# caizexin/GenVC

Measured on AMD Instinct MI355X. Metric: utterances/s (streaming, 1 s chunks; with RTF and first-chunk latency), higher is better.
Workload: dtype f32; 1 GPU; GenVC_small streaming, 1 s chunks, top_k=1, batch 1 per GPU (BASELINE configs[1]); parallelism=replicas x1, utterances sharded by rank, all_gather of token ids

## Files before the change

genvc_amd/csrc/attn64.h:

```cpp
#pragma once
#include "gemm.h"

namespace gvc {

typedef float hb_f32x4 __attribute__((ext_vector_type(4)));

template <bool MASK, int NW = 4>
__global__ __launch_bounds__(NW * 64) void k_attn64_mfma(const float* qb, const float* kb, const float* vb, long long ld, long long bs, int Tq,
                                                     int Tk, float* out, int out_rows, int E, float scale, int out_fm16, const int32_t* fmask) {
    __shared__ float sm[NW][16], sl[NW][16];
    __shared__ __attribute__((aligned(16))) float so[NW][16][68];
    const int tid = threadIdx.x, lane = tid & 63, wave = tid >> 6, r = lane & 15, g = lane >> 4;
    const int q0 = blockIdx.x * 16, h = blockIdx.y, b = blockIdx.z;
    const float* base = qb + (size_t)b * bs + h * 64;
    const float* kbase = kb + (size_t)b * bs + h * 64;
    const float* vbase = vb + (size_t)b * bs + h * 64;
    const int T = Tk;
    const int qi = min(q0 + r, Tq - 1);
    float4 qf[4];
#pragma unroll
    for (int s = 0; s < 4; ++s) {
        qf[s] = *reinterpret_cast<const float4*>(base + (size_t)qi * ld + 16 * s + 4 * g);
        qf[s].x *= scale; qf[s].y *= scale; qf[s].z *= scale; qf[s].w *= scale;
    }
// ... 58 lines not shown
        *reinterpret_cast<float4*>(&so[wave][r][16 * g + 4 * i]) = make_float4(o[0][i], o[1][i], o[2][i], o[3][i]);
    __syncthreads();
    const int qr = tid >> 4, dc = (tid & 15) * 4;
    if (tid < 256 && q0 + qr < Tq) {
        float M = sm[0][qr];
#pragma unroll
        for (int w = 1; w < NW; ++w) M = fmaxf(M, sm[w][qr]);
        float L = 0.f;
        float4 acc = make_float4(0.f, 0.f, 0.f, 0.f);
#pragma unroll
        for (int w = 0; w < NW; ++w) {
            const float f = sm[w][qr] == -INFINITY ? 0.f : expf(sm[w][qr] - M);
            L += sl[w][qr] * f;
            const float4 ov = *reinterpret_cast<const float4*>(&so[w][qr][dc]);
            acc.x += ov.x * f; acc.y += ov.y * f; acc.z += ov.z * f; acc.w += ov.w * f;
        }
        const float inv = 1.0f / L;
        acc.x *= inv; acc.y *= inv; acc.z *= inv; acc.w *= inv;
        if (out_fm16) *reinterpret_cast<float4*>(out + fm16_index(b * out_rows + q0 + qr, h * 64 + dc, E)) = acc;
        else *reinterpret_cast<float4*>(out + ((size_t)b * out_rows + q0 + qr) * E + h * 64 + dc) = acc;
    }
}

}
```

genvc_amd/csrc/gemm.h:

```cpp
#pragma once
#include "common.h"

namespace gvc {

__host__ __device__ __forceinline__ size_t fm16_index(int m, int k, int K) {
    return ((size_t)(m >> 4) * (K >> 4) + (k >> 4)) * 256 + (size_t)((((m & 15) + 16 * ((k & 15) >> 2)) << 2) + (k & 3));
}

enum GemmAct { ACT_NONE = 0, ACT_GELU_NEW = 1, ACT_RELU = 2, ACT_GELU_ERF = 3 };
enum GemmAAct { AACT_NONE = 0, AACT_LRELU = 1 };

struct GemmEpi {
    const float* bias;
    long long bias_batch_stride;
    int act;
    const float* resid;
    int ldr;
    long long resid_batch_stride;
    long long resid_batch_stride2;
    int resid_fm16;
    int geglu;
    const float* resid2;
    float out_scale;
    int c_fm16;
// ... 188 lines not shown
    *reinterpret_cast<float4*>(G.C + (size_t)m * G.ldc + n) = v;
}

typedef float f32x16 __attribute__((ext_vector_type(16)));

__global__ __launch_bounds__(256) void k_gemm_f32(const GemmArgs G);
__global__ void k_splitk_epilogue(const GemmArgs G);

int launch_gemm_skinny(GemmArgs G, int SK, long long work_cap, hipStream_t s);
int launch_ln_sum_rows(const float* x_in, float* x_out, float* a, const float* part, int SK, const float* bias, int rows, int d,
                       const float* ln_w, const float* ln_b, int a_fm16, hipStream_t s);
struct LnFuse {
    const float* x_in; float* x_out;
    const float* part; int SK; const float* pbias;
    const float* ln_w; const float* ln_b;
    int rows;
};
int launch_gemm_skinny_ln(GemmArgs G, const LnFuse& P, hipStream_t s);
int launch_gemm_strip(GemmArgs G, int sk_max, long long work_cap, int raw_partials, int* sk_used, hipStream_t s);
void gemm_init_attributes();
__global__ void k_to_fm16(const float* src, float* dst, int N, int K);
__global__ void k_to_fm16_bf16(const float* src, unsigned short* dst, int N, int K);

int launch_gemm_cap(GemmArgs G, int batch, long long work_cap, hipStream_t s);

}
```

genvc_amd/csrc/gemm.hip:

```cpp
#include "gemm.h"
#include "gemm_b16.h"
#include <algorithm>

namespace gvc {

constexpr int BM = 64, BN = 64, BK = 32, LDL = 36;

__global__ __launch_bounds__(256) void k_gemm_f32(const GemmArgs G) {
    __shared__ __attribute__((aligned(16))) float As[2][BM * LDL];
    __shared__ __attribute__((aligned(16))) float Bs[2][BN * LDL];
    const int tid = threadIdx.x, lane = tid & 63, wave = tid >> 6;
    const int wm = wave >> 1, wn = wave & 1;
    const int batch = blockIdx.z / G.SK, sk = blockIdx.z - batch * G.SK;
    const int m0 = blockIdx.y * BM, n0 = blockIdx.x * BN;
    const int ntile_all = (G.K + BK - 1) / BK;
    const int tps = (ntile_all + G.SK - 1) / G.SK;
    const int kbeg = sk * tps * BK;
    const int kend = min(G.K, kbeg + tps * BK);
    const int nt = kend > kbeg ? (kend - kbeg + BK - 1) / BK : 0;
    const float* Ab = G.A + gemm_boff(G, batch, G.a_batch_stride, G.a_batch_stride2);
    const float* Wb = G.Wt + gemm_binner(G, batch) * G.w_batch_stride;

    float4 ra[2], rb[2];
    auto load_tile = [&](int kt) {
// ... 64 lines not shown
                G.work[(((size_t)batch * G.SK + sk) * G.M + m) * G.N + n] = acc[r];
            else
                gemm_store(G, batch, m, n, acc[r]);
        }
    }
}

__global__ void k_splitk_epilogue(const GemmArgs G) {
    const int batch = blockIdx.z;
    const size_t mn = (size_t)G.M * G.N;
    for (size_t i = (size_t)blockIdx.x * blockDim.x + threadIdx.x; i < mn; i += (size_t)gridDim.x * blockDim.x) {
        const float* w = G.work + (size_t)batch * G.SK * mn + i;
        float pv[16];
#pragma unroll
        for (int s = 0; s < 16; ++s) pv[s] = w[(size_t)min(s, G.SK - 1) * mn];
        float v = 0.f;
#pragma unroll
        for (int s = 0; s < 16; ++s)
            if (s < G.SK) v += pv[s];
        gemm_store(G, batch, (int)(i / G.N), (int)(i % G.N), v);
    }
}

int launch_gemm_cap(GemmArgs G, int batch, long long work_cap, hipStream_t s) {
    GVC_REQUIRE(G.K % 4 == 0 && G.lda % 4 == 0 && G.ldw % 4 == 0 && G.conv_cin % 4 == 0 && G.conv_tap_stride % 4 == 0,
                GVC_ERR_ARG, "gemm: K/lda/ldw/conv strides must be multiples of 4 (K=%d lda=%d ldw=%d)", G.K, G.lda, G.ldw);
    const int tm = cdiv(G.M, BM), tn = cdiv(G.N, BN);
    const long long tiles = (long long)tm * tn * batch;
    int SK = 1;
    constexpr int sk_tiles = 128, sk_target = 192;
    if (tiles < sk_tiles && G.work) {
        SK = (int)((sk_target + tiles - 1) / tiles);
        const int max_by_k = G.K / (4 * BK) > 0 ? G.K / (4 * BK) : 1;
        if (SK > max_by_k) SK = max_by_k;
        if (SK > 16) SK = 16;
        while (SK > 1 && (long long)batch * SK * G.M * G.N > work_cap) --SK;
    } else if (tiles < 2 * sk_tiles && G.K >= 64 * BK && G.work) {
        SK = (int)((4 * sk_tiles + tiles - 1) / tiles);
        if (SK > G.K / (16 * BK)) SK = G.K / (16 * BK);
        while (SK > 1 && (long long)batch * SK * G.M * G.N > work_cap) --SK;
    }
    G.SK = SK;
    dim3 grid(tn, tm, batch * SK);
    hipLaunchKernelGGL(k_gemm_f32, grid, dim3(256), 0, s, G);
    GVC_LAUNCH_CHECK();
    if (SK > 1) {
        const long long mn = (long long)G.M * G.N;
        int gx = (int)((mn + 255) / 256);
        if (gx > 2048) gx = 2048;
        hipLaunchKernelGGL(k_splitk_epilogue, dim3(gx, 1, batch), dim3(256), 0, s, G);
        GVC_LAUNCH_CHECK();
    }
    return GVC_OK;
}

typedef float f32x4 __attribute__((ext_vector_type(4)));

template <int WB> struct WRaw { typedef float4 T; };
template <> struct WRaw<1> { typedef uint2 T; };
__device__ __forceinline__ float4 w_f4(const float4& r) { return r; }
__device__ __forceinline__ float4 w_f4(const uint2& u) {
    return make_float4(__uint_as_float(u.x << 16), __uint_as_float(u.x & 0xffff0000u), __uint_as_float(u.y << 16),
                       __uint_as_float(u.y & 0xffff0000u));
}

template <int MT, int NW, int WB = 0, int NC = 0>
__global__ __launch_bounds__(NW * 64) void k_gemm_skinny(const GemmArgs G) {
    extern __shared__ __attribute__((aligned(16))) float red_raw[];
    float (*red)[MT][256] = reinterpret_cast<float (*)[MT][256]>(red_raw);
// ... 775 lines not shown
```

genvc_amd/csrc/hubert.hip:

```cpp
#include <map>
#include <string>
#include <vector>

#include "conv_lds.h"
#include "attn64.h"
#include <algorithm>

namespace gvc {

constexpr int kC0Chunk = 32;

static __global__ void k_hb_repack_conv(const float* w, float* out, int Co, int Ci, int k) {
    const size_t n = (size_t)Co * Ci * k;
    for (size_t i = (size_t)blockIdx.x * blockDim.x + threadIdx.x; i < n; i += (size_t)gridDim.x * blockDim.x) {
        const int j = (int)(i % k);
        const int ci = (int)((i / k) % Ci);
        const int co = (int)(i / ((size_t)k * Ci));
        out[((size_t)co * k + j) * Ci + ci] = w[i];
    }
}

static __global__ __launch_bounds__(256) void k_hb_conv0(const float* wav, const float* w, float* y, float* part, int T,
                                                        int T0, int C, int k, int stride) {
    extern __shared__ float xs[];
    const int b = blockIdx.z, chunk = blockIdx.x, tid = threadIdx.x;
    const int t0 = chunk * kC0Chunk;
    const int nt = min(kC0Chunk, T0 - t0);
    const int nx = (nt - 1) * stride + k;
    const float* src = wav + (size_t)b * T + (size_t)t0 * stride;
    for (int i = tid; i < nx; i += 256) xs[i] = src[i];
    __syncthreads();
    for (int c = blockIdx.y * 256 + tid; c < min(C, (int)(blockIdx.y + 1) * 256); c += 256) {
        float wr[16];
// ... 39 lines not shown
    const double mean = s / T0;
    double var = ss / T0 - mean * mean;
    if (var < 0.0) var = 0.0;
    stats[((size_t)b * C + c) * 2] = (float)mean;
    stats[((size_t)b * C + c) * 2 + 1] = (float)(1.0 / sqrt(var + 1e-5));
}

static __global__ void k_hb_gn_gelu(float* y, const float* stats, const float* gamma, const float* beta, int T0, int C) {
    const int b = blockIdx.y;
    const size_t n4 = (size_t)T0 * C / 4;
    float* yb = y + (size_t)b * T0 * C;
    for (size_t i = (size_t)blockIdx.x * blockDim.x + threadIdx.x; i < n4; i += (size_t)gridDim.x * blockDim.x) {
        const int c = (int)((i * 4) % C);
        float4 v = *reinterpret_cast<float4*>(yb + i * 4);
        const float* st = stats + ((size_t)b * C + c) * 2;
        v.x = gelu_erf((v.x - st[0]) * st[1] * gamma[c] + beta[c]);
        v.y = gelu_erf((v.y - st[2]) * st[3] * gamma[c + 1] + beta[c + 1]);
        v.z = gelu_erf((v.z - st[4]) * st[5] * gamma[c + 2] + beta[c + 2]);
        v.w = gelu_erf((v.w - st[6]) * st[7] * gamma[c + 3] + beta[c + 3]);
        *reinterpret_cast<float4*>(yb + i * 4) = v;
    }
}

static __global__ __launch_bounds__(256) void k_hb_ln_rows(const float* src, long long src_bs, float* dst, long long dst_bs,
                                                          int rpb, int d, const float* w, const float* b,
                                                          const float* part = nullptr, int SK = 0, const float* pbias = nullptr,
                                                          int rows = 0, float* dst_fm16 = nullptr) {
    __shared__ float red[4];
    const int row = blockIdx.x, tid = threadIdx.x;
    const int bi = row / rpb, ri = row - bi * rpb;
    const float* xr = src + bi * src_bs + (size_t)ri * d;
    float* orow = dst + bi * dst_bs + (size_t)ri * d;
    float4 v[4];
    float s = 0.f;
#pragma unroll
    for (int i = 0; i < 4; ++i) {
        const int k = (i * 256 + tid) * 4;
        v[i] = k < d ? *reinterpret_cast<const float4*>(xr + k) : make_float4(0.f, 0.f, 0.f, 0.f);
        if (part && k < d) {
            const float4 b4 = *reinterpret_cast<const float4*>(pbias + k);
            float4 p4[8];
#pragma unroll
            for (int sidx = 0; sidx < 8; ++sidx)
                p4[sidx] = *reinterpret_cast<const float4*>(part + ((size_t)min(sidx, SK - 1) * rows + row) * d + k);
            v[i].x += b4.x; v[i].y += b4.y; v[i].z += b4.z; v[i].w += b4.w;
#pragma unroll
            for (int sidx = 0; sidx < 8; ++sidx)
                if (sidx < SK) { v[i].x += p4[sidx].x; v[i].y += p4[sidx].y; v[i].z += p4[sidx].z; v[i].w += p4[sidx].w; }
        }
        s += (v[i].x + v[i].y) + (v[i].z + v[i].w);
    }
    const float inv_d = 1.0f / (float)d;
    const float mean = block4_sum(s, red) * inv_d;
    float q = 0.f;
#pragma unroll
    for (int i = 0; i < 4; ++i) {
        const int k = (i * 256 + tid) * 4;
        if (k < d) {
            const float a0 = v[i].x - mean, a1 = v[i].y - mean, a2 = v[i].z - mean, a3 = v[i].w - mean;
            q += (a0 * a0 + a1 * a1) + (a2 * a2 + a3 * a3);
        }
    }
    const float rstd = 1.0f / sqrtf(block4_sum(q, red) * inv_d + 1e-5f);
#pragma unroll
    for (int i = 0; i < 4; ++i) {
        const int k = (i * 256 + tid) * 4;
        if (k < d) {
            const float4 gw = *reinterpret_cast<const float4*>(w + k);
            const float4 gb = *reinterpret_cast<const float4*>(b + k);
            float4 o;
// ... 7 lines not shown

static __global__ void k_hb_zero_pad(float* buf, int C, int T, int front, int back, const int32_t* fmask) {
    const int b = blockIdx.y;
    float* base = buf + (size_t)b * (front + T + back) * C;
    const size_t nf = (size_t)front * C, nb = (size_t)back * C;
    for (size_t i = (size_t)blockIdx.x * blockDim.x + threadIdx.x; i < nf + nb; i += (size_t)gridDim.x * blockDim.x) {
        if (i < nf) base[i] = 0.f;
        else base[(size_t)(front + T) * C + (i - nf)] = 0.f;
    }
    for (int t = blockIdx.x; t < T; t += gridDim.x) {
        if (!fmask[b * T + t]) continue;
        for (int i = threadIdx.x; i < C; i += blockDim.x) base[(size_t)(front + t) * C + i] = 0.f;
    }
}

static __global__ __launch_bounds__(64) void k_hb_frame_mask(const float* wav, int32_t* fmask, int T, int F) {
    const int f = blockIdx.x, b = blockIdx.y, lane = threadIdx.x;
    const int chunk = T / F;
    const float* p = wav + (size_t)b * T + (size_t)f * chunk;
    int nz = 0;
    for (int i = lane; i < chunk; i += 64) nz |= (p[i] != 0.f);
    nz = __any(nz);
    if (lane == 0) fmask[b * F + f] = nz ? 0 : 1;
}

}

using namespace gvc;

struct HbLin { float* w = nullptr; float* b = nullptr; int N = 0, K = 0; float* wf = nullptr;  };
struct HbLn { float* w = nullptr; float* b = nullptr; };
struct HbLayer { HbLin qkv, out, fc1, fc2; HbLn ln1, ln2; };

struct gvc_hubert {
    gvc_hubert_dims dm;
    int cg = 0, pad_front = 0, pad_back = 0;
    float* conv0_w = nullptr;
    HbLn gn;
    std::vector<float*> conv_w;
    std::vector<float*> conv_wp;
    int conv_lds = 1;
    int conv_lds_rows = 256;
    HbLn feat_ln, enc_ln;
    HbLin proj, pos, fin;
    std::vector<HbLayer> layers;
    std::map<std::string, int> bound;
    int n_expected = 0;
    float *act[2] = {nullptr, nullptr};
    float *part = nullptr, *stats = nullptr;
    int32_t* fmask = nullptr;
    float *xp = nullptr, *x = nullptr, *qkv = nullptr, *att = nullptr, *hbuf = nullptr, *tmp = nullptr, *work = nullptr;
    long long work_cap = 0;
    int max_frames = 0, max_t0 = 0;
    std::map<long long, hipGraphExec_t> graphs;
    hipStream_t cap_stream = nullptr;
    int use_graph = 1;
    int skinny = 1;
    int strip = 1;
    bool fm_ready = false;
    float *xf = nullptr, *af = nullptr, *hf = nullptr;
    std::vector<void*> allocs;
};

static int hb_alloc(gvc_hubert* c, float** p, size_t n) {
    GVC_CHECK_HIP(hipMalloc((void**)p, n * sizeof(float)));
    c->allocs.push_back(*p);
    return GVC_OK;
}
static int hb_alloc_lin(gvc_hubert* c, HbLin& L, int N, int K) {
    L.N = N; L.K = K;
    int rc = hb_alloc(c, &L.w, (size_t)N * K);
    return rc ? rc : hb_alloc(c, &L.b, N);
}
static int hb_alloc_ln(gvc_hubert* c, HbLn& L, int d) {
    int rc = hb_alloc(c, &L.w, d);
    return rc ? rc : hb_alloc(c, &L.b, d);
}

static int hb_frames(const gvc_hubert_dims& D, int n, int upto) {
    for (int i = 0; i < upto; ++i) {
        if (n < D.conv_kernel[i]) return 0;
// ... 42 lines not shown
                conv_lds_bytes(D.conv_dim[i - 1], D.conv_kernel[i], 1, false, D.conv_stride[i]) <= kConvLdsMax)
                rc = hb_alloc(c, &wp, (size_t)D.conv_dim[i] * D.conv_kernel[i] * D.conv_dim[i - 1]);
            c->conv_wp.push_back(wp);
        }
    }
    const int Cl = D.conv_dim[D.n_conv - 1];
    if (!rc) rc = hb_alloc_ln(c, c->feat_ln, Cl);
    if (!rc) rc = hb_alloc_lin(c, c->proj, E, Cl);
    if (!rc) rc = hb_alloc_lin(c, c->pos, E, kp * c->cg);
    if (!rc) rc = hb_alloc_ln(c, c->enc_ln, E);
    c->layers.resize(D.n_layers);
    for (int l = 0; l < D.n_layers && !rc; ++l) {
        HbLayer& L = c->layers[l];
        if ((rc = hb_alloc_lin(c, L.qkv, 3 * E, E))) break;
        if ((rc = hb_alloc_lin(c, L.out, E, E))) break;
        if ((rc = hb_alloc_lin(c, L.fc1, D.ffn_dim, E))) break;
        if ((rc = hb_alloc_lin(c, L.fc2, E, D.ffn_dim))) break;
        if ((rc = hb_alloc_ln(c, L.ln1, E))) break;
        if ((rc = hb_alloc_ln(c, L.ln2, E))) break;
        for (HbLin* q : {&L.qkv, &L.out, &L.fc1, &L.fc2})
            if ((rc = hb_alloc(c, &q->wf, (size_t)q->N * q->K))) break;
    }
    if (!rc) rc = hb_alloc_lin(c, c->fin, D.final_dim, E);
    c->n_expected = 3 + (D.n_conv - 1) + 2 + 2 + 2 + 2 + 16 * D.n_layers + 2;
    const size_t B = D.max_batch, F = c->max_frames;
    for (int i = 0; i < 2 && !rc; ++i) rc = hb_alloc(c, &c->act[i], B * maxact);
    if (!rc) rc = hb_alloc(c, &c->part, B * (size_t)cdiv(c->max_t0, kC0Chunk) * D.conv_dim[0] * 2);
    if (!rc) rc = hb_alloc(c, &c->stats, B * D.conv_dim[0] * 2);
    if (!rc) rc = hb_alloc(c, reinterpret_cast<float**>(&c->fmask), B * F);
    if (!rc) rc = hb_alloc(c, &c->xp, B * (F + kp) * E);
    if (!rc) rc = hb_alloc(c, &c->x, B * F * E);
    if (!rc) rc = hb_alloc(c, &c->tmp, B * F * E);
    if (!rc) rc = hb_alloc(c, &c->att, B * F * E);
    if (!rc) rc = hb_alloc(c, &c->qkv, B * F * 3 * E);
    if (!rc) rc = hb_alloc(c, &c->hbuf, B * F * D.ffn_dim);
    const size_t fm_rows = std::max<size_t>(128, (B * F + 15) & ~(size_t)15);
    if (!rc) rc = hb_alloc(c, &c->xf, fm_rows * E);
    if (!rc) rc = hb_alloc(c, &c->af, fm_rows * E);
    if (!rc) rc = hb_alloc(c, &c->hf, fm_rows * D.ffn_dim);
    c->work_cap = 16ll << 20;
    if (!rc) rc = hb_alloc(c, &c->work, (size_t)c->work_cap);
    if (!rc && hipStreamCreateWithFlags(&c->cap_stream, hipStreamNonBlocking) != hipSuccess) rc = GVC_ERR_HIP;
    if (getenv("GVC_GRAPHS")) c->use_graph = atoi(getenv("GVC_GRAPHS"));
    conv_lds_init_attributes();
    if (E % 128 != 0 || D.ffn_dim % 128 != 0) c->skinny = 0;
    if (rc) { gvc_hubert_destroy(c); return rc; }
    *out = c;
    return GVC_OK;
}

extern "C" int gvc_hubert_destroy(gvc_hubert* c) {
    if (!c) return GVC_OK;
    for (auto& kv : c->graphs) hipGraphExecDestroy(kv.second);
    if (c->cap_stream) hipStreamDestroy(c->cap_stream);
    for (void* p : c->allocs) hipFree(p);
    delete c;
    return GVC_OK;
}

static int hb_copy(float* dst, const float* src, int64_t numel, int64_t expect, const char* name, hipStream_t s) {
    GVC_REQUIRE(numel == expect, GVC_ERR_ARG, "%s: expected %lld elements, got %lld", name, (long long)expect, (long long)numel);
    GVC_CHECK_HIP(hipMemcpyAsync(dst, src, numel * sizeof(float), hipMemcpyDeviceToDevice, s));
    return GVC_OK;
}

static bool ends_with(const std::string& n, const char* suf) {
// ... 42 lines not shown
        HbLayer& L = c->layers[l];
        const size_t dot = n.find('.', 15);
        const std::string sub = n.substr(dot + 1);
        int which = -1;
        if (sub.rfind("self_attn.q_proj.", 0) == 0) which = 0;
        else if (sub.rfind("self_attn.k_proj.", 0) == 0) which = 1;
        else if (sub.rfind("self_attn.v_proj.", 0) == 0) which = 2;
        if (which >= 0) {
            if (is_b) rc = hb_copy(L.qkv.b + (size_t)which * E, src, numel, E, name, s);
            else rc = hb_copy(L.qkv.w + (size_t)which * E * E, src, numel, (int64_t)E * E, name, s);
        } else if (sub.rfind("self_attn.out_proj.", 0) == 0) rc = lin(L.out);
        else if (sub.rfind("self_attn_layer_norm.", 0) == 0) rc = ln(L.ln1, E);
        else if (sub.rfind("fc1.", 0) == 0) rc = lin(L.fc1);
        else if (sub.rfind("fc2.", 0) == 0) rc = lin(L.fc2);
        else if (sub.rfind("final_layer_norm.", 0) == 0) rc = ln(L.ln2, E);
        else known = false;
    } else known = false;
    if (rc == GVC_OK && known) { c->bound[n] = 1; c->fm_ready = false; }
    return rc;
}

extern "C" int gvc_hubert_missing_weights(gvc_hubert* c) { return c ? c->n_expected - (int)c->bound.size() : -1; }

static int hb_linear(gvc_hubert* c, const HbLin& L, const float* A, float* C, int M, int act, const float* resid, hipStream_t s) {
    GemmArgs G;
    memset(&G, 0, sizeof(G));
    G.A = A; G.lda = L.K; G.Wt = L.w; G.ldw = L.K; G.C = C; G.ldc = L.N;
    G.M = M; G.N = L.N; G.K = L.K; G.work = c->work;
    G.e.bias = L.b; G.e.act = act;
    if (resid) { G.e.resid = resid; G.e.ldr = L.N; }
    return launch_gemm_cap(G, 1, c->work_cap, s);
}

static int hb_body(gvc_hubert* c, int B, int T, hipStream_t s) {
    const gvc_hubert_dims& D = c->dm;
    const int E = D.embed_dim;
    int rc;
    int Tin = hb_frames(D, T, 1);
    const int C0 = D.conv_dim[0];
    const int nchunk = cdiv(Tin, kC0Chunk);
    hipLaunchKernelGGL(k_hb_gn_stats, dim3(cdiv(C0, 8), B), dim3(256), 0, s, c->part, c->stats, nchunk, Tin, C0);
    GVC_LAUNCH_CHECK();
    {
        const size_t n4 = (size_t)Tin * C0 / 4;
        const int gx = (int)std::min<size_t>((n4 + 255) / 256, 4096);
        hipLaunchKernelGGL(k_hb_gn_gelu, dim3(gx, B), dim3(256), 0, s, c->act[0], c->stats, c->gn.w, c->gn.b, Tin, C0);
        GVC_LAUNCH_CHECK();
    }
    int cur = 0;
    for (int i = 1; i < D.n_conv; ++i) {
        const int Ci = D.conv_dim[i - 1], Co = D.conv_dim[i], k = D.conv_kernel[i], st = D.conv_stride[i];
        const int Tout = (Tin - k) / st + 1;
        if (c->conv_lds && c->conv_wp[i - 1] && Tout <= c->conv_lds_rows) {
            ConvLdsArgs A;
            memset(&A, 0, sizeof(A));
            A.x = c->act[cur]; A.x_bs = (long long)Tin * Ci; A.ldx = Ci; A.x_scale = 1.f; A.slope = 1.f;
            A.x_rows = Tin; A.stride = st;
            A.y = c->act[cur ^ 1]; A.y_bs = (long long)Tout * Co; A.ldy = Co;
            A.T = Tout; A.ntiles = Co / 16; A.act = ACT_GELU_ERF;
            A.job[0].wp = reinterpret_cast<const float4*>(c->conv_wp[i - 1]); A.job[0].k = k; A.job[0].dil = 1;
            if ((rc = launch_conv_lds(Ci, 1, A, 1, B, conv_lds_bytes(Ci, k, 1, false, st), s))) return rc;
            cur ^= 1;
            Tin = Tout;
            continue;
        }
        GemmArgs G;
        memset(&G, 0, sizeof(G));
        G.A = c->act[cur]; G.lda = st * Ci; G.a_batch_stride = (long long)Tin * Ci;
        G.Wt = c->conv_w[i - 1]; G.ldw = k * Ci;
        G.C = c->act[cur ^ 1]; G.ldc = Co; G.c_batch_stride = (long long)Tout * Co;
        G.M = Tout; G.N = Co; G.K = k * Ci; G.work = c->work;
        G.e.act = ACT_GELU_ERF;
        if ((rc = launch_gemm_cap(G, B, c->work_cap, s))) return rc;
        cur ^= 1;
        Tin = Tout;
    }
    const int F = Tin, Cl = D.conv_dim[D.n_conv - 1], rows = B * F;
    const int kp = D.pos_conv_kernel;
    const long long xp_bs = (long long)(F + kp - 1) * E;
    hipLaunchKernelGGL(k_hb_ln_rows, dim3(rows), dim3(256), 0, s, c->act[cur], (long long)F * Cl, c->act[cur ^ 1],
                       (long long)F * Cl, F, Cl, c->feat_ln.w, c->feat_ln.b);
    GVC_LAUNCH_CHECK();
    {
        GemmArgs G;
        memset(&G, 0, sizeof(G));
        G.A = c->act[cur ^ 1]; G.lda = Cl; G.a_batch_stride = (long long)F * Cl;
        G.Wt = c->proj.w; G.ldw = Cl;
        G.C = c->xp + (size_t)c->pad_front * E; G.ldc = E; G.c_batch_stride = xp_bs;
        G.M = F; G.N = E; G.K = Cl; G.work = c->work;
        G.e.bias = c->proj.b;
        if ((rc = launch_gemm_cap(G, B, c->work_cap, s))) return rc;
    }
    hipLaunchKernelGGL(k_hb_zero_pad, dim3(64, B), dim3(256), 0, s, c->xp, E, F, c->pad_front, c->pad_back, c->fmask);
    GVC_LAUNCH_CHECK();
    {
        GemmArgs G;
        memset(&G, 0, sizeof(G));
        const int cg = c->cg;
        G.batch_inner = D.pos_conv_groups;
        G.A = c->xp; G.lda = E; G.a_batch_stride = cg; G.a_batch_stride2 = xp_bs;
        G.conv_cin = cg; G.conv_tap_stride = E;
        G.Wt = c->pos.w; G.ldw = kp * cg; G.w_batch_stride = (long long)cg * kp * cg;
        G.C = c->tmp; G.ldc = E; G.c_batch_stride = cg; G.c_batch_stride2 = (long long)F * E;
        G.M = F; G.N = cg; G.K = kp * cg; G.work = c->work;
        G.e.bias = c->pos.b; G.e.bias_batch_stride = cg; G.e.act = ACT_GELU_ERF;
        G.e.resid = c->xp + (size_t)c->pad_front * E; G.e.ldr = E; G.e.resid_batch_stride = cg; G.e.resid_batch_stride2 = xp_bs;
        if ((rc = launch_gemm_cap(G, B * D.pos_conv_groups, c->work_cap, s))) return rc;
    }
    const bool skinny = c->skinny && (rows <= 128 || (c->strip && E % 64 == 0 && D.ffn_dim % 64 == 0));
    const bool strip = rows > 128;
    if (skinny) {
        hipLaunchKernelGGL(k_hb_ln_rows, dim3(rows), dim3(256), 0, s, c->tmp, (long long)F * E, c->x, (long long)F * E, F, E,
                           c->enc_ln.w, c->enc_ln.b, (const float*)nullptr, 0, (const float*)nullptr, rows, c->xf);
        GVC_LAUNCH_CHECK();
        int sk_used = 1;
        auto sk_gemm = [&](const HbLin& L, const float* A_fm, float* C, int act, int c_fm16, int SK, const float* resid = nullptr) {
            GemmArgs G;
            memset(&G, 0, sizeof(G));
            G.A = A_fm; G.lda = L.K; G.Wt = L.wf; G.ldw = L.K; G.C = C; G.ldc = L.N; G.M = rows; G.N = L.N; G.K = L.K;
            G.work = c->work;
            if (strip && resid) {
                if ((long long)rows * L.N > c->work_cap) { set_error("hubert: %d rows exceed the split-K work buffer", rows); return (int)GVC_ERR_ARG; }
                return launch_gemm_strip(G, 8, c->work_cap, 1, &sk_used, s);
            }
            sk_used = SK;
            if (SK == 1) { G.e.bias = L.b; G.e.act = act; G.e.c_fm16 = c_fm16; G.e.resid = resid; G.e.ldr = L.N; }
            if (strip) return launch_gemm_strip(G, 1, c->work_cap, 0, nullptr, s);
            return launch_gemm_skinny(G, SK, c->work_cap, s);
        };
        auto post_ln = [&](const HbLin& L, const HbLn& N, int) {
            const int SK = sk_used;
            if (SK > 1 || strip)
                hipLaunchKernelGGL(k_hb_ln_rows, dim3(rows), dim3(256), 0, s, c->x, (long long)F * E, c->x, (long long)F * E, F, E,
                                   N.w, N.b, c->work, SK, L.b, rows, c->xf);
            else
                hipLaunchKernelGGL(k_hb_ln_rows, dim3(rows), dim3(256), 0, s, c->tmp, (long long)F * E, c->x, (long long)F * E, F, E,
                                   N.w, N.b, (const float*)nullptr, 0, (const float*)nullptr, rows, c->xf);
        };
        const int sk_out = (E / 2) % 128 == 0 ? 2 : 1, sk_fc2 = (D.ffn_dim / 4) % 128 == 0 ? 4 : ((D.ffn_dim / 2) % 128 == 0 ? 2 : 1);
        for (int l = 0; l < D.n_layers; ++l) {
            const HbLayer& L = c->layers[l];
            if ((rc = sk_gemm(L.qkv, c->xf, c->qkv, ACT_NONE, 0, 1))) return rc;
            hipLaunchKernelGGL(k_attn64_mfma<true>, dim3(cdiv(F, 16), D.n_heads, B), dim3(256), 0, s, c->qkv, c->qkv + E, c->qkv + 2 * E, (long long)3 * E, (long long)F * 3 * E, F, F, c->af, F, E, 0.125f, 1, c->fmask);
            GVC_LAUNCH_CHECK();
            if ((rc = sk_gemm(L.out, c->af, c->tmp, ACT_NONE, 0, sk_out, c->x))) return rc;
            post_ln(L.out, L.ln1, sk_out);
            GVC_LAUNCH_CHECK();
            if ((rc = sk_gemm(L.fc1, c->xf, c->hf, ACT_GELU_ERF, 1, 1))) return rc;
            if ((rc = sk_gemm(L.fc2, c->hf, c->tmp, ACT_NONE, 0, sk_fc2, c->x))) return rc;
            post_ln(L.fc2, L.ln2, sk_fc2);
            GVC_LAUNCH_CHECK();
        }
        return GVC_OK;
    }
    hipLaunchKernelGGL(k_hb_ln_rows, dim3(rows), dim3(256), 0, s, c->tmp, (long long)F * E, c->x, (long long)F * E, F, E,
                       c->enc_ln.w, c->enc_ln.b);
    GVC_LAUNCH_CHECK();
    for (int l = 0; l < D.n_layers; ++l) {
        const HbLayer& L = c->layers[l];
        if ((rc = hb_linear(c, L.qkv, c->x, c->qkv, rows, ACT_NONE, nullptr, s))) return rc;
        hipLaunchKernelGGL(k_attn64_mfma<true>, dim3(cdiv(F, 16), D.n_heads, B), dim3(256), 0, s, c->qkv, c->qkv + E, c->qkv + 2 * E, (long long)3 * E, (long long)F * 3 * E, F, F, c->att, F, E, 0.125f, 0, c->fmask);
        GVC_LAUNCH_CHECK();
        if ((rc = hb_linear(c, L.out, c->att, c->tmp, rows, ACT_NONE, c->x, s))) return rc;
        hipLaunchKernelGGL(k_hb_ln_rows, dim3(rows), dim3(256), 0, s, c->tmp, (long long)F * E, c->x, (long long)F * E, F, E,
                           L.ln1.w, L.ln1.b);
        GVC_LAUNCH_CHECK();
        if ((rc = hb_linear(c, L.fc1, c->x, c->hbuf, rows, ACT_GELU_ERF, nullptr, s))) return rc;
        if ((rc = hb_linear(c, L.fc2, c->hbuf, c->tmp, rows, ACT_NONE, c->x, s))) return rc;
        hipLaunchKernelGGL(k_hb_ln_rows, dim3(rows), dim3(256), 0, s, c->tmp, (long long)F * E, c->x, (long long)F * E, F, E,
                           L.ln2.w, L.ln2.b);
        GVC_LAUNCH_CHECK();
    }
    return GVC_OK;
}

extern "C" int gvc_hubert_forward(gvc_hubert* c, const float* wav, int32_t B, int32_t T, float* out, gvc_stream sv) {
    GVC_REQUIRE(c && wav && out, GVC_ERR_ARG, "gvc_hubert_forward: null argument");
    GVC_REQUIRE(gvc_hubert_missing_weights(c) == 0, GVC_ERR_STATE, "%d HuBERT weight tensors are not bound",
                gvc_hubert_missing_weights(c));
    const gvc_hubert_dims& D = c->dm;
    const int F = hb_frames(D, T, D.n_conv);
    GVC_REQUIRE(B >= 1 && B <= D.max_batch && T <= D.max_samples && F >= 1, GVC_ERR_ARG,
                "hubert: B=%d samples=%d outside capacity (%d, %d) or too short", B, T, D.max_batch, D.max_samples);
    hipStream_t s = (hipStream_t)sv;
    if (c->skinny && !c->fm_ready) {
        for (HbLayer& L : c->layers)
            for (HbLin* q : {&L.qkv, &L.out, &L.fc1, &L.fc2}) {
                hipLaunchKernelGGL(k_to_fm16, dim3(1024), dim3(256), 0, s, q->w, q->wf, q->N, q->K);
                GVC_LAUNCH_CHECK();
            }
        c->fm_ready = true;
    }
    const int T0 = hb_frames(D, T, 1), C0 = D.conv_dim[0], k0 = D.conv_kernel[0], s0 = D.conv_stride[0];
    hipLaunchKernelGGL(k_hb_conv0, dim3(cdiv(T0, kC0Chunk), cdiv(C0, 256), B), dim3(256), ((kC0Chunk - 1) * s0 + k0) * sizeof(float), s, wav,
                       c->conv0_w, c->act[0], c->part, T, T0, C0, k0, s0);
    GVC_LAUNCH_CHECK();
    hipLaunchKernelGGL(k_hb_frame_mask, dim3(F, B), dim3(64), 0, s, wav, c->fmask, T, F);
    GVC_LAUNCH_CHECK();
    int rc;
    if (!c->use_graph) {
        if ((rc = hb_body(c, B, T, s))) return rc;
    } else {
        const long long key = ((long long)B << 32) | (unsigned)T;
        auto it = c->graphs.find(key);
        if (it == c->graphs.end()) {
            if (c->graphs.size() >= 64) {
                for (auto& kv : c->graphs) hipGraphExecDestroy(kv.second);
                c->graphs.clear();
            }
            hipGraphExec_t ge;
            if ((rc = capture_graph(c->cap_stream, &ge, [&] { return hb_body(c, B, T, c->cap_stream); }))) return rc;
            it = c->graphs.emplace(key, ge).first;
        }
        GVC_CHECK_HIP(hipGraphLaunch(it->second, s));
    }
    {
        GemmArgs G;
        memset(&G, 0, sizeof(G));
        const HbLin& L = c->fin;
        G.A = c->x; G.lda = L.K; G.Wt = L.w; G.ldw = L.K; G.C = out; G.ldc = L.N;
        G.M = B * F; G.N = L.N; G.K = L.K; G.work = c->work;
        G.e.bias = L.b;
        if ((rc = launch_gemm_cap(G, 1, c->work_cap, s))) return rc;
    }
    return GVC_OK;
}
```

Before: 7.048 utterances/s.

## Fold HuBERT attention out-projection, split-K reductions, and final proj into fewer kernels

Adds a fused attention kernel that computes per-head output projection partials directly into a work plane, then reduces them together with bias and residual inside the post-attention LayerNorm. Folds the proj GEMM split-K reduction into the zero-pad kernel and the pos-conv split-K partials into the encoder LayerNorm. The final projection now uses the skinny fm16 GEMM path. The intent is to cut kernel launches and intermediate round trips for small streaming chunks. In exchange, each head writes its own partial plane and the split-K reductions become wider.

```diff
diff --git a/genvc_amd/csrc/attn64.h b/genvc_amd/csrc/attn64.h
--- a/genvc_amd/csrc/attn64.h
+++ b/genvc_amd/csrc/attn64.h
@@ -104,4 +104,141 @@
     }
 }
 
+template <bool MASK>
+__global__ __launch_bounds__(256) void k_attn64_outproj(const float* qb, const float* kb, const float* vb, long long ld, long long bs, int Tq,
+                                                        int Tk, const float* wf, float* plane, int out_rows, int rows, int E, int ncb,
+                                                        float scale, const int32_t* fmask) {
+    constexpr int NW = 4;
+    __shared__ float sm[NW][16], sl[NW][16];
+    __shared__ __attribute__((aligned(16))) float so[NW][16][68];
+    const int tid = threadIdx.x, lane = tid & 63, wave = tid >> 6, r = lane & 15, g = lane >> 4;
+    const int qt = blockIdx.x / ncb, cb = blockIdx.x - qt * ncb;
+    const int q0 = qt * 16, h = blockIdx.y, b = blockIdx.z;
+    const int K16 = E >> 4, ntpb = (K16 + ncb - 1) / ncb;
+    float4 wfr[3][4];
+    bool wok[3];
+    auto request_weights = [&]() {
+#pragma unroll
+        for (int j = 0; j < 3; ++j) {
+            const int nt = cb * ntpb + wave + 4 * j;
+            wok[j] = wave + 4 * j < ntpb && nt < K16;
+            const float4* wp = reinterpret_cast<const float4*>(wf) + ((size_t)(wok[j] ? nt : 0) * K16 + 4 * h) * 64 + lane;
+#pragma unroll
+            for (int s = 0; s < 4; ++s) wfr[j][s] = wp[s * 64];
+        }
+    };
+    const float* base = qb + (size_t)b * bs + h * 64;
+    const float* kbase = kb + (size_t)b * bs + h * 64;
+    const float* vbase = vb + (size_t)b * bs + h * 64;
+    const int T = Tk;
+    const int qi = min(q0 + r, Tq - 1);
+    float4 qf[4];
+#pragma unroll
+    for (int s = 0; s < 4; ++s) {
+        qf[s] = *reinterpret_cast<const float4*>(base + (size_t)qi * ld + 16 * s + 4 * g);
+        qf[s].x *= scale; qf[s].y *= scale; qf[s].z *= scale; qf[s].w *= scale;
+    }
+    hb_f32x4 o[4];
+#pragma unroll
+    for (int mt = 0; mt < 4; ++mt) o[mt] = {0.f, 0.f, 0.f, 0.f};
+    float m = -INFINITY, l = 0.f;
+    const int ntile = (T + 15) >> 4;
+    for (int kt = wave; kt < ntile; kt += NW) {
+        const int key0 = kt * 16;
+        const int kr = min(key0 + r, T - 1);
+        float4 kf[4], vf[4];
+#pragma unroll
+        for (int s = 0; s < 4; ++s) kf[s] = *reinterpret_cast<const float4*>(kbase + (size_t)kr * ld + 16 * s + 4 * g);
+        int kmask[4];
+#pragma unroll
+        for (int i = 0; i < 4; ++i) {
+            const int vr = min(key0 + 4 * g + i, T - 1);
+            vf[i] = *reinterpret_cast<const float4*>(vbase + (size_t)vr * ld + 4 * r);
+            kmask[i] = MASK ? fmask[b * T + vr] : 0;
+        }
+        if (kt == wave) request_weights();
+        hb_f32x4 st = {0.f, 0.f, 0.f, 0.f};
+#pragma unroll
+        for (int s = 0; s < 4; ++s) {
+            st = __builtin_amdgcn_mfma_f32_16x16x4f32(kf[s].x, qf[s].x, st, 0, 0, 0);
+            st = __builtin_amdgcn_mfma_f32_16x16x4f32(kf[s].y, qf[s].y, st, 0, 0, 0);
+            st = __builtin_amdgcn_mfma_f32_16x16x4f32(kf[s].z, qf[s].z, st, 0, 0, 0);
+            st = __builtin_amdgcn_mfma_f32_16x16x4f32(kf[s].w, qf[s].w, st, 0, 0, 0);
+        }
+        float p[4];
+        float tmax = -INFINITY;
+#pragma unroll
+        for (int i = 0; i < 4; ++i) {
+            p[i] = (key0 + 4 * g + i < T && !kmask[i]) ? st[i] : -INFINITY;
+            tmax = fmaxf(tmax, p[i]);
+        }
+        tmax = fmaxf(tmax, __shfl_xor(tmax, 16));
+        tmax = fmaxf(tmax, __shfl_xor(tmax, 32));
+        const float mnew = fmaxf(m, tmax);
+        const bool none = mnew == -INFINITY;
+        const float alpha = none ? 1.0f : expf(m - mnew);
+        float psum = 0.f;
+#pragma unroll
+        for (int i = 0; i < 4; ++i) { p[i] = none ? 0.f : expf(p[i] - mnew); psum += p[i]; }
+        l = l * alpha + psum;
+#pragma unroll
+        for (int mt = 0; mt < 4; ++mt) o[mt] *= alpha;
+#pragma unroll
+        for (int i = 0; i < 4; ++i) {
+            o[0] = __builtin_amdgcn_mfma_f32_16x16x4f32(vf[i].x, p[i], o[0], 0, 0, 0);
+            o[1] = __builtin_amdgcn_mfma_f32_16x16x4f32(vf[i].y, p[i], o[1], 0, 0, 0);
+            o[2] = __builtin_amdgcn_mfma_f32_16x16x4f32(vf[i].z, p[i], o[2], 0, 0, 0);
+            o[3] = __builtin_amdgcn_mfma_f32_16x16x4f32(vf[i].w, p[i], o[3], 0, 0, 0);
+        }
+        m = mnew;
+    }
+    if (wave >= ntile) request_weights();
+    l += __shfl_xor(l, 16);
+    l += __shfl_xor(l, 32);
+    if (g == 0) { sm[wave][r] = m; sl[wave][r] = l; }
+#pragma unroll
+    for (int i = 0; i < 4; ++i)
+        *reinterpret_cast<float4*>(&so[wave][r][16 * g + 4 * i]) = make_float4(o[0][i], o[1][i], o[2][i], o[3][i]);
+    __syncthreads();
+    {
+        const int qr = tid >> 4, dc = (tid & 15) * 4;
+        float M = sm[0][qr];
+#pragma unroll
+        for (int w = 1; w < NW; ++w) M = fmaxf(M, sm[w][qr]);
+        float L = 0.f;
+        float4 acc = make_float4(0.f, 0.f, 0.f, 0.f);
+#pragma unroll
+        for (int w = 0; w < NW; ++w) {
+            const float f = sm[w][qr] == -INFINITY ? 0.f : expf(sm[w][qr] - M);
+            L += sl[w][qr] * f;
+            const float4 ov = *reinterpret_cast<const float4*>(&so[w][qr][dc]);
+            acc.x += ov.x * f; acc.y += ov.y * f; acc.z += ov.z * f; acc.w += ov.w * f;
+        }
+        const float inv = 1.0f / L;
+        acc.x *= inv; acc.y *= inv; acc.z *= inv; acc.w *= inv;
+        *reinterpret_cast<float4*>(&so[0][qr][dc]) = acc;
+    }
+    __syncthreads();
+    float4 af[4];
+#pragma unroll
+    for (int s = 0; s < 4; ++s) af[s] = *reinterpret_cast<const float4*>(&so[0][r][16 * s + 4 * g]);
+    float* prow = plane + ((size_t)h * rows + (size_t)b * out_rows + q0 + 4 * g) * E;
+#pragma unroll
+    for (int j = 0; j < 3; ++j) {
+        if (!wok[j]) continue;
+        hb_f32x4 c = {0.f, 0.f, 0.f, 0.f};
+#pragma unroll
+        for (int s = 0; s < 4; ++s) {
+            c = __builtin_amdgcn_mfma_f32_16x16x4f32(af[s].x, wfr[j][s].x, c, 0, 0, 0);
+            c = __builtin_amdgcn_mfma_f32_16x16x4f32(af[s].y, wfr[j][s].y, c, 0, 0, 0);
+            c = __builtin_amdgcn_mfma_f32_16x16x4f32(af[s].z, wfr[j][s].z, c, 0, 0, 0);
+            c = __builtin_amdgcn_mfma_f32_16x16x4f32(af[s].w, wfr[j][s].w, c, 0, 0, 0);
+        }
+        const int n = (cb * ntpb + wave + 4 * j) * 16 + r;
+#pragma unroll
+        for (int i = 0; i < 4; ++i)
+            if (q0 + 4 * g + i < Tq) prow[(size_t)i * E + n] = c[i];
+    }
 }
+
+}
diff --git a/genvc_amd/csrc/gemm.h b/genvc_amd/csrc/gemm.h
--- a/genvc_amd/csrc/gemm.h
+++ b/genvc_amd/csrc/gemm.h
@@ -234,6 +234,6 @@
 __global__ void k_to_fm16(const float* src, float* dst, int N, int K);
 __global__ void k_to_fm16_bf16(const float* src, unsigned short* dst, int N, int K);
 
-int launch_gemm_cap(GemmArgs G, int batch, long long work_cap, hipStream_t s);
-
-}
+int launch_gemm_cap(GemmArgs G, int batch, long long work_cap, hipStream_t s, int* raw_sk = nullptr);
+
+}
diff --git a/genvc_amd/csrc/gemm.hip b/genvc_amd/csrc/gemm.hip
--- a/genvc_amd/csrc/gemm.hip
+++ b/genvc_amd/csrc/gemm.hip
@@ -110,7 +110,7 @@
     }
 }
 
-int launch_gemm_cap(GemmArgs G, int batch, long long work_cap, hipStream_t s) {
+int launch_gemm_cap(GemmArgs G, int batch, long long work_cap, hipStream_t s, int* raw_sk) {
     GVC_REQUIRE(G.K % 4 == 0 && G.lda % 4 == 0 && G.ldw % 4 == 0 && G.conv_cin % 4 == 0 && G.conv_tap_stride % 4 == 0,
                 GVC_ERR_ARG, "gemm: K/lda/ldw/conv strides must be multiples of 4 (K=%d lda=%d ldw=%d)", G.K, G.lda, G.ldw);
     const int tm = cdiv(G.M, BM), tn = cdiv(G.N, BN);
@@ -132,7 +132,8 @@
     dim3 grid(tn, tm, batch * SK);
     hipLaunchKernelGGL(k_gemm_f32, grid, dim3(256), 0, s, G);
     GVC_LAUNCH_CHECK();
-    if (SK > 1) {
+    if (raw_sk) *raw_sk = SK;
+    if (SK > 1 && !raw_sk) {
         const long long mn = (long long)G.M * G.N;
         int gx = (int)((mn + 255) / 256);
         if (gx > 2048) gx = 2048;
diff --git a/genvc_amd/csrc/hubert.hip b/genvc_amd/csrc/hubert.hip
--- a/genvc_amd/csrc/hubert.hip
+++ b/genvc_amd/csrc/hubert.hip
@@ -9,6 +9,16 @@
 namespace gvc {
 
 constexpr int kC0Chunk = 32;
+
+enum HbFold {
+    kFoldProjPad = 1,
+    kFoldPosLn = 2,
+    kFoldFinal = 4,
+    kFoldAttnOut = 8,
+};
+#ifndef GVC_HB_FOLDS
+#define GVC_HB_FOLDS 15
+#endif
 
 static __global__ void k_hb_repack_conv(const float* w, float* out, int Co, int Ci, int k) {
     const size_t n = (size_t)Co * Ci * k;
@@ -94,10 +104,11 @@
     }
 }
 
+template <int NP, bool POS>
 static __global__ __launch_bounds__(256) void k_hb_ln_rows(const float* src, long long src_bs, float* dst, long long dst_bs,
                                                           int rpb, int d, const float* w, const float* b,
                                                           const float* part = nullptr, int SK = 0, const float* pbias = nullptr,
-                                                          int rows = 0, float* dst_fm16 = nullptr) {
+                                                          int rows = 0, float* dst_fm16 = nullptr, int cg = 0) {
     __shared__ float red[4];
     const int row = blockIdx.x, tid = threadIdx.x;
     const int bi = row / rpb, ri = row - bi * rpb;
@@ -109,15 +120,35 @@
     for (int i = 0; i < 4; ++i) {
         const int k = (i * 256 + tid) * 4;
         v[i] = k < d ? *reinterpret_cast<const float4*>(xr + k) : make_float4(0.f, 0.f, 0.f, 0.f);
-        if (part && k < d) {
+        if constexpr (POS) {
+            if (k < d) {
+                const float4 b4 = *reinterpret_cast<const float4*>(pbias + k);
+                const int grp = k / cg;
+                const size_t pstride = (size_t)rpb * cg;
+                const float* p0 = part + ((size_t)(bi * (d / cg) + grp) * SK * rpb + ri) * cg + (k - grp * cg);
+                float4 p4[NP];
+#pragma unroll
+                for (int sidx = 0; sidx < NP; ++sidx) p4[sidx] = *reinterpret_cast<const float4*>(p0 + (size_t)min(sidx, SK - 1) * pstride);
+                float4 a = make_float4(0.f, 0.f, 0.f, 0.f);
+#pragma unroll
+                for (int sidx = 0; sidx < NP; ++sidx)
+                    if (sidx < SK) { a.x += p4[sidx].x; a.y += p4[sidx].y; a.z += p4[sidx].z; a.w += p4[sidx].w; }
+                a.x += b4.x; a.y += b4.y; a.z += b4.z; a.w += b4.w;
+                {
+#pragma clang fp contract(off)
+                    v[i].x = gelu_erf(a.x) + v[i].x; v[i].y = gelu_erf(a.y) + v[i].y;
+                    v[i].z = gelu_erf(a.z) + v[i].z; v[i].w = gelu_erf(a.w) + v[i].w;
+                }
+            }
+        } else if (part && k < d) {
             const float4 b4 = *reinterpret_cast<const float4*>(pbias + k);
-            float4 p4[8];
-#pragma unroll
-            for (int sidx = 0; sidx < 8; ++sidx)
+            float4 p4[NP];
+#pragma unroll
+            for (int sidx = 0; sidx < NP; ++sidx)
                 p4[sidx] = *reinterpret_cast<const float4*>(part + ((size_t)min(sidx, SK - 1) * rows + row) * d + k);
             v[i].x += b4.x; v[i].y += b4.y; v[i].z += b4.z; v[i].w += b4.w;
 #pragma unroll
-            for (int sidx = 0; sidx < 8; ++sidx)
+            for (int sidx = 0; sidx < NP; ++sidx)
                 if (sidx < SK) { v[i].x += p4[sidx].x; v[i].y += p4[sidx].y; v[i].z += p4[sidx].z; v[i].w += p4[sidx].w; }
         }
         s += (v[i].x + v[i].y) + (v[i].z + v[i].w);
@@ -171,6 +202,29 @@
     for (int i = lane; i < chunk; i += 64) nz |= (p[i] != 0.f);
     nz = __any(nz);
     if (lane == 0) fmask[b * F + f] = nz ? 0 : 1;
+}
+
+static __global__ __launch_bounds__(256) void k_hb_proj_finish(const float* work, int SK, const float* bias, float* xp, int E, int T,
+                                                              int front, int back, const int32_t* fmask) {
+    const int b = blockIdx.y, row = blockIdx.x, t = row - front;
+    float* dst = xp + ((size_t)b * (front + T + back) + row) * E;
+    const bool live = t >= 0 && t < T && !fmask[b * T + min(max(t, 0), T - 1)];
+    const size_t mn = (size_t)T * E;
+    for (int k = threadIdx.x * 4; k < E; k += 256 * 4) {
+        float4 v = make_float4(0.f, 0.f, 0.f, 0.f);
+        if (live) {
+            const float* w = work + (size_t)b * SK * mn + (size_t)t * E + k;
+            float4 pv[16];
+#pragma unroll
+            for (int s = 0; s < 16; ++s) pv[s] = *reinterpret_cast<const float4*>(w + (size_t)min(s, SK - 1) * mn);
+            const float4 b4 = *reinterpret_cast<const float4*>(bias + k);
+#pragma unroll
+            for (int s = 0; s < 16; ++s)
+                if (s < SK) { v.x += pv[s].x; v.y += pv[s].y; v.z += pv[s].z; v.w += pv[s].w; }
+            v.x += b4.x; v.y += b4.y; v.z += b4.z; v.w += b4.w;
+        }
+        *reinterpret_cast<float4*>(dst + k) = v;
+    }
 }
 
 }
@@ -206,6 +260,7 @@
     int use_graph = 1;
     int skinny = 1;
     int strip = 1;
+    int folds = GVC_HB_FOLDS;
     bool fm_ready = false;
     float *xf = nullptr, *af = nullptr, *hf = nullptr;
     std::vector<void*> allocs;
@@ -294,6 +349,7 @@
             if ((rc = hb_alloc(c, &q->wf, (size_t)q->N * q->K))) break;
     }
     if (!rc) rc = hb_alloc_lin(c, c->fin, D.final_dim, E);
+    if (!rc && D.final_dim % 16 == 0 && E % 64 == 0) rc = hb_alloc(c, &c->fin.wf, (size_t)D.final_dim * E);
     c->n_expected = 3 + (D.n_conv - 1) + 2 + 2 + 2 + 2 + 16 * D.n_layers + 2;
     const size_t B = D.max_batch, F = c->max_frames;
     for (int i = 0; i < 2 && !rc; ++i) rc = hb_alloc(c, &c->act[i], B * maxact);
@@ -313,7 +369,11 @@
     c->work_cap = 16ll << 20;
     if (!rc) rc = hb_alloc(c, &c->work, (size_t)c->work_cap);
     if (!rc && hipStreamCreateWithFlags(&c->cap_stream, hipStreamNonBlocking) != hipSuccess) rc = GVC_ERR_HIP;
-    if (getenv("GVC_GRAPHS")) c->use_graph = atoi(getenv("GVC_GRAPHS"));
+    if (getenv("GVC_GRAPHS")) {
+        const int v = atoi(getenv("GVC_GRAPHS"));
+        c->use_graph = v != 0 && v != 2;
+        if (v == 2) c->folds = 0;
+    }
     conv_lds_init_attributes();
     if (E % 128 != 0 || D.ffn_dim % 128 != 0) c->skinny = 0;
     if (rc) { gvc_hubert_destroy(c); return rc; }
@@ -402,6 +462,8 @@
 
 extern "C" int gvc_hubert_missing_weights(gvc_hubert* c) { return c ? c->n_expected - (int)c->bound.size() : -1; }
 
+static bool hb_skinny_rows(const gvc_hubert* c, int rows) { return c->skinny && rows <= 128; }
+
 static int hb_linear(gvc_hubert* c, const HbLin& L, const float* A, float* C, int M, int act, const float* resid, hipStream_t s) {
     GemmArgs G;
     memset(&G, 0, sizeof(G));
@@ -419,6 +481,7 @@
     int Tin = hb_frames(D, T, 1);
     const int C0 = D.conv_dim[0];
     const int nchunk = cdiv(Tin, kC0Chunk);
+    const bool small = hb_skinny_rows(c, B * hb_frames(D, T, D.n_conv));
     hipLaunchKernelGGL(k_hb_gn_stats, dim3(cdiv(C0, 8), B), dim3(256), 0, s, c->part, c->stats, nchunk, Tin, C0);
     GVC_LAUNCH_CHECK();
     {
@@ -458,7 +521,7 @@
     const int F = Tin, Cl = D.conv_dim[D.n_conv - 1], rows = B * F;
     const int kp = D.pos_conv_kernel;
     const long long xp_bs = (long long)(F + kp - 1) * E;
-    hipLaunchKernelGGL(k_hb_ln_rows, dim3(rows), dim3(256), 0, s, c->act[cur], (long long)F * Cl, c->act[cur ^ 1],
+    hipLaunchKernelGGL((k_hb_ln_rows<8, false>), dim3(rows), dim3(256), 0, s, c->act[cur], (long long)F * Cl, c->act[cur ^ 1],
                        (long long)F * Cl, F, Cl, c->feat_ln.w, c->feat_ln.b);
     GVC_LAUNCH_CHECK();
     {
@@ -469,10 +532,17 @@
         G.C = c->xp + (size_t)c->pad_front * E; G.ldc = E; G.c_batch_stride = xp_bs;
         G.M = F; G.N = E; G.K = Cl; G.work = c->work;
         G.e.bias = c->proj.b;
-        if ((rc = launch_gemm_cap(G, B, c->work_cap, s))) return rc;
-    }
-    hipLaunchKernelGGL(k_hb_zero_pad, dim3(64, B), dim3(256), 0, s, c->xp, E, F, c->pad_front, c->pad_back, c->fmask);
-    GVC_LAUNCH_CHECK();
+        int sk = 1;
+        const bool fold = small && (c->folds & kFoldProjPad);
+        if ((rc = launch_gemm_cap(G, B, c->work_cap, s, fold ? &sk : nullptr))) return rc;
+        if (fold && sk > 1)
+            hipLaunchKernelGGL(k_hb_proj_finish, dim3(c->pad_front + F + c->pad_back, B), dim3(256), 0, s, c->work, sk, c->proj.b, c->xp, E, F,
+                               c->pad_front, c->pad_back, c->fmask);
+        else
+            hipLaunchKernelGGL(k_hb_zero_pad, dim3(64, B), dim3(256), 0, s, c->xp, E, F, c->pad_front, c->pad_back, c->fmask);
+        GVC_LAUNCH_CHECK();
+    }
+    int pos_sk = 1;
     {
         GemmArgs G;
         memset(&G, 0, sizeof(G));
@@ -485,13 +555,17 @@
         G.M = F; G.N = cg; G.K = kp * cg; G.work = c->work;
         G.e.bias = c->pos.b; G.e.bias_batch_stride = cg; G.e.act = ACT_GELU_ERF;
         G.e.resid = c->xp + (size_t)c->pad_front * E; G.e.ldr = E; G.e.resid_batch_stride = cg; G.e.resid_batch_stride2 = xp_bs;
-        if ((rc = launch_gemm_cap(G, B * D.pos_conv_groups, c->work_cap, s))) return rc;
+        if ((rc = launch_gemm_cap(G, B * D.pos_conv_groups, c->work_cap, s, small && (c->folds & kFoldPosLn) ? &pos_sk : nullptr))) return rc;
     }
     const bool skinny = c->skinny && (rows <= 128 || (c->strip && E % 64 == 0 && D.ffn_dim % 64 == 0));
     const bool strip = rows > 128;
     if (skinny) {
-        hipLaunchKernelGGL(k_hb_ln_rows, dim3(rows), dim3(256), 0, s, c->tmp, (long long)F * E, c->x, (long long)F * E, F, E,
-                           c->enc_ln.w, c->enc_ln.b, (const float*)nullptr, 0, (const float*)nullptr, rows, c->xf);
+        if (pos_sk > 1)
+            hipLaunchKernelGGL((k_hb_ln_rows<16, true>), dim3(rows), dim3(256), 0, s, c->xp + (size_t)c->pad_front * E, xp_bs, c->x,
+                               (long long)F * E, F, E, c->enc_ln.w, c->enc_ln.b, c->work, pos_sk, c->pos.b, rows, c->xf, c->cg);
+        else
+            hipLaunchKernelGGL((k_hb_ln_rows<8, false>), dim3(rows), dim3(256), 0, s, c->tmp, (long long)F * E, c->x, (long long)F * E, F, E,
+                               c->enc_ln.w, c->enc_ln.b, (const float*)nullptr, 0, (const float*)nullptr, rows, c->xf);
         GVC_LAUNCH_CHECK();
         int sk_used = 1;
         auto sk_gemm = [&](const HbLin& L, const float* A_fm, float* C, int act, int c_fm16, int SK, const float* resid = nullptr) {
@@ -511,21 +585,32 @@
         auto post_ln = [&](const HbLin& L, const HbLn& N, int) {
             const int SK = sk_used;
             if (SK > 1 || strip)
-                hipLaunchKernelGGL(k_hb_ln_rows, dim3(rows), dim3(256), 0, s, c->x, (long long)F * E, c->x, (long long)F * E, F, E,
+                hipLaunchKernelGGL((k_hb_ln_rows<8, false>), dim3(rows), dim3(256), 0, s, c->x, (long long)F * E, c->x, (long long)F * E, F, E,
                                    N.w, N.b, c->work, SK, L.b, rows, c->xf);
             else
-                hipLaunchKernelGGL(k_hb_ln_rows, dim3(rows), dim3(256), 0, s, c->tmp, (long long)F * E, c->x, (long long)F * E, F, E,
+                hipLaunchKernelGGL((k_hb_ln_rows<8, false>), dim3(rows), dim3(256), 0, s, c->tmp, (long long)F * E, c->x, (long long)F * E, F, E,
                                    N.w, N.b, (const float*)nullptr, 0, (const float*)nullptr, rows, c->xf);
         };
+        const int ncb = std::max(4, cdiv(E / 16, 12));
+        const bool attn_out = !strip && (c->folds & kFoldAttnOut) && D.n_heads <= 16 && (long long)D.n_heads * rows * E <= c->work_cap;
         const int sk_out = (E / 2) % 128 == 0 ? 2 : 1, sk_fc2 = (D.ffn_dim / 4) % 128 == 0 ? 4 : ((D.ffn_dim / 2) % 128 == 0 ? 2 : 1);
         for (int l = 0; l < D.n_layers; ++l) {
             const HbLayer& L = c->layers[l];
             if ((rc = sk_gemm(L.qkv, c->xf, c->qkv, ACT_NONE, 0, 1))) return rc;
-            hipLaunchKernelGGL(k_attn64_mfma<true>, dim3(cdiv(F, 16), D.n_heads, B), dim3(256), 0, s, c->qkv, c->qkv + E, c->qkv + 2 * E, (long long)3 * E, (long long)F * 3 * E, F, F, c->af, F, E, 0.125f, 1, c->fmask);
-            GVC_LAUNCH_CHECK();
-            if ((rc = sk_gemm(L.out, c->af, c->tmp, ACT_NONE, 0, sk_out, c->x))) return rc;
-            post_ln(L.out, L.ln1, sk_out);
-            GVC_LAUNCH_CHECK();
+            if (attn_out) {
+                hipLaunchKernelGGL(k_attn64_outproj<true>, dim3(cdiv(F, 16) * ncb, D.n_heads, B), dim3(256), 0, s, c->qkv, c->qkv + E, c->qkv + 2 * E,
+                                   (long long)3 * E, (long long)F * 3 * E, F, F, L.out.wf, c->work, F, rows, E, ncb, 0.125f, c->fmask);
+                GVC_LAUNCH_CHECK();
+                hipLaunchKernelGGL((k_hb_ln_rows<16, false>), dim3(rows), dim3(256), 0, s, c->x, (long long)F * E, c->x, (long long)F * E, F, E,
+                                   L.ln1.w, L.ln1.b, c->work, D.n_heads, L.out.b, rows, c->xf);
+                GVC_LAUNCH_CHECK();
+            } else {
+                hipLaunchKernelGGL(k_attn64_mfma<true>, dim3(cdiv(F, 16), D.n_heads, B), dim3(256), 0, s, c->qkv, c->qkv + E, c->qkv + 2 * E, (long long)3 * E, (long long)F * 3 * E, F, F, c->af, F, E, 0.125f, 1, c->fmask);
+                GVC_LAUNCH_CHECK();
+                if ((rc = sk_gemm(L.out, c->af, c->tmp, ACT_NONE, 0, sk_out, c->x))) return rc;
+                post_ln(L.out, L.ln1, sk_out);
+                GVC_LAUNCH_CHECK();
+            }
             if ((rc = sk_gemm(L.fc1, c->xf, c->hf, ACT_GELU_ERF, 1, 1))) return rc;
             if ((rc = sk_gemm(L.fc2, c->hf, c->tmp, ACT_NONE, 0, sk_fc2, c->x))) return rc;
             post_ln(L.fc2, L.ln2, sk_fc2);
@@ -533,7 +618,7 @@
         }
         return GVC_OK;
     }
-    hipLaunchKernelGGL(k_hb_ln_rows, dim3(rows), dim3(256), 0, s, c->tmp, (long long)F * E, c->x, (long long)F * E, F, E,
+    hipLaunchKernelGGL((k_hb_ln_rows<8, false>), dim3(rows), dim3(256), 0, s, c->tmp, (long long)F * E, c->x, (long long)F * E, F, E,
                        c->enc_ln.w, c->enc_ln.b);
     GVC_LAUNCH_CHECK();
     for (int l = 0; l < D.n_layers; ++l) {
@@ -542,12 +627,12 @@
         hipLaunchKernelGGL(k_attn64_mfma<true>, dim3(cdiv(F, 16), D.n_heads, B), dim3(256), 0, s, c->qkv, c->qkv + E, c->qkv + 2 * E, (long long)3 * E, (long long)F * 3 * E, F, F, c->att, F, E, 0.125f, 0, c->fmask);
         GVC_LAUNCH_CHECK();
         if ((rc = hb_linear(c, L.out, c->att, c->tmp, rows, ACT_NONE, c->x, s))) return rc;
-        hipLaunchKernelGGL(k_hb_ln_rows, dim3(rows), dim3(256), 0, s, c->tmp, (long long)F * E, c->x, (long long)F * E, F, E,
+        hipLaunchKernelGGL((k_hb_ln_rows<8, false>), dim3(rows), dim3(256), 0, s, c->tmp, (long long)F * E, c->x, (long long)F * E, F, E,
                            L.ln1.w, L.ln1.b);
         GVC_LAUNCH_CHECK();
         if ((rc = hb_linear(c, L.fc1, c->x, c->hbuf, rows, ACT_GELU_ERF, nullptr, s))) return rc;
         if ((rc = hb_linear(c, L.fc2, c->hbuf, c->tmp, rows, ACT_NONE, c->x, s))) return rc;
-        hipLaunchKernelGGL(k_hb_ln_rows, dim3(rows), dim3(256), 0, s, c->tmp, (long long)F * E, c->x, (long long)F * E, F, E,
+        hipLaunchKernelGGL((k_hb_ln_rows<8, false>), dim3(rows), dim3(256), 0, s, c->tmp, (long long)F * E, c->x, (long long)F * E, F, E,
                            L.ln2.w, L.ln2.b);
         GVC_LAUNCH_CHECK();
     }
@@ -569,6 +654,10 @@
                 hipLaunchKernelGGL(k_to_fm16, dim3(1024), dim3(256), 0, s, q->w, q->wf, q->N, q->K);
                 GVC_LAUNCH_CHECK();
             }
+        if (c->fin.wf) {
+            hipLaunchKernelGGL(k_to_fm16, dim3(1024), dim3(256), 0, s, c->fin.w, c->fin.wf, c->fin.N, c->fin.K);
+            GVC_LAUNCH_CHECK();
+        }
         c->fm_ready = true;
     }
     const int T0 = hb_frames(D, T, 1), C0 = D.conv_dim[0], k0 = D.conv_kernel[0], s0 = D.conv_stride[0];
@@ -594,7 +683,15 @@
         }
         GVC_CHECK_HIP(hipGraphLaunch(it->second, s));
     }
-    {
+    const HbLin& Lf = c->fin;
+    if ((c->folds & kFoldFinal) && hb_skinny_rows(c, B * F) && Lf.wf && Lf.K % 64 == 0) {
+        GemmArgs G;
+        memset(&G, 0, sizeof(G));
+        G.A = c->xf; G.lda = Lf.K; G.Wt = Lf.wf; G.ldw = Lf.K; G.C = out; G.ldc = Lf.N;
+        G.M = B * F; G.N = Lf.N; G.K = Lf.K; G.work = c->work;
+        G.e.bias = Lf.b; G.e.ldr = Lf.N;
+        if ((rc = launch_gemm_skinny(G, 1, c->work_cap, s))) return rc;
+    } else {
         GemmArgs G;
         memset(&G, 0, sizeof(G));
         const HbLin& L = c->fin;
```

After: 7.088 utterances/s (median of 6 runs). About the same (+0.6%).
